# SebLague/Ray-Tracing

Hardware: AMD Instinct MI355X
Metric: Mrays/s at 1920x1080, 8 spp, 8 bounces; per-channel L2 vs reference (higher is better)
Workload: dtype f32

## Files before the change

### ray-tracing_amd/csrc/rt_context.hip

```cpp
#include <hip/hip_runtime.h>

#include <math.h>
#include <stdarg.h>
#include <stdio.h>
#include <stdlib.h>
#include <string.h>
#include <dlfcn.h>
#include <sys/mman.h>

#include <cmath>
#include <string>
#include <vector>

#include <algorithm>
#include <atomic>
#include <chrono>
#include <mutex>
#include <thread>
#include <unordered_map>

#include "rt_kernels.h"
#include "../../include/rt_cost.h"
#include "../../include/rt_aov.h"
#include "../../include/rt_denoise.h"
#include "../../include/rt_reproject.h"

#include "rt_denoise_launch.h"
#include "rt_denoise_math.h"
#include "rt_reproject_launch.h"
#include "rt_layout.h"
#include "rt_launch_order.h"
#include "rt_launch_plan.h"
#define RT_VERSION_STRING "raytrace_hip gfx950 abi=1"

static thread_local char g_err[512] = "";

struct RtContext;
struct LaunchJob;
struct HipOrder final : rt_order::Backend {
    RtContext* ctx = nullptr;
    hipEvent_t ev[rt_order::EVENT_COUNT] = {};
    LaunchJob* job = nullptr;
    hipStream_t stream(int s) const;
    int record(rt_order::Event e, int s) override;
// ... 87 lines not shown
    struct Tuner {
        int decided = 3;
        bool done = false;
        double ms[2] = {0, 0};
        int n[2] = {0, 0};
        int next = 0;
        struct Probe { hipEvent_t start = nullptr, stop = nullptr; int cand = 0, frames = 0; bool live = false; } probe[6];
    } tuner;
    float* dStaging[2] = {nullptr, nullptr};
    size_t stagingBytes[2] = {0, 0};
    bool stagingUnavailable = false;
    bool alternateWanted = true;
    rt_order::LaunchOrder order;
    HipOrder backend;
    int lastLaunched = 0;
    void* dDisplay = nullptr;
    void* dAovOut = nullptr;
    size_t aovOutBytes = 0;
    unsigned long long* dAovWords = nullptr;
    bool aovUnreported = false;
    void* dDnScratch = nullptr;
    size_t dnScratchBytes = 0;
    void* dDnAov = nullptr;
    size_t dnAovBytes = 0;
    size_t displayBytes = 0;
    hipEvent_t evStart = nullptr, evStop = nullptr;
    double gpuMs = 0;
    int timerState = 0;
};

// ... 145 lines not shown
        HIP_TRY(ctx, hipMalloc(&ctx->dTileQueue, 2 * sizeof(unsigned long long)));
        HIP_TRY(ctx, hipMemsetAsync(ctx->dTileQueue, 0, 2 * sizeof(unsigned long long), ctx->ownStream));
        HIP_TRY(ctx, hipStreamSynchronize(ctx->ownStream));
        HIP_TRY(ctx, hipEventCreate(&ctx->evStart));
        HIP_TRY(ctx, hipEventCreate(&ctx->evStop));
        for (hipEvent_t& ev : ctx->backend.ev) HIP_TRY(ctx, hipEventCreateWithFlags(&ev, hipEventDisableTiming));
        return RT_OK;
    };
    if (int rc = init()) {
        rt_destroy(ctx);
        return rc;
    }
    memset(&ctx->params, 0, sizeof(ctx->params));
    if (const char* g = getenv("RT_GRID")) ctx->gridOverride = atoi(g);
    if (const char* g = getenv("RT_POOL_MIN_ITEMS")) ctx->poolMinItems = atoi(g);
    if (const char* g = getenv("RT_POOL_FAULT")) { if (atoi(g)) ctx->poolSpinLimit = 64u | 0x80000000u; }
    if (getenv("RT_VERBOSE")) ctx->verbose = true;
    if (const char* f = getenv("RT_FUSE_FRAMES")) ctx->fuseFrames = atoi(f) != 0;
    if (const char* l = getenv("RT_LPT")) ctx->order.lpt = atoi(l) != 0;
    if (const char* t = getenv("RT_TWO_STREAMS")) ctx->twoStreams = atoi(t) != 0;
    if (const char* c = getenv("RT_COALESCE")) ctx->coalesce = atoi(c) != 0;
    if (const char* fg = getenv("RT_FRAME_GROUP")) ctx->frameGroupOverride = atoi(fg);
    if (const char* al = getenv("RT_ALTERNATE")) ctx->order.alternate = ctx->alternateWanted = atoi(al) != 0;
    ctx->order.set_two_streams(ctx->twoStreams && ctx->sideStream);
    if (const char* fc = getenv("RT_FUSE_CAP"))
        if (const int cap = rt_plan::pinned_fuse_cap(atoi(fc))) { ctx->fuseCap = cap; ctx->fuseCapPinned = true; }
    *out = ctx;
    return RT_OK;
}

// ... 13 lines not shown
    ctx->haveScene = false;
}

void rt_destroy(RtContext* ctx)
{
    if (!ctx) return;
    hipSetDevice(ctx->device);
    flush_pending(ctx);
    if (ctx->sideStream) hipStreamSynchronize(ctx->sideStream);
    hipStreamSynchronize(ctx->stream);
    free_scene(ctx);
    hipFree(ctx->ownFrame);
    hipFree(ctx->ownAccum);
    hipFree(ctx->dCounters);
    hipFree(ctx->dTileQueue);
    hipFree(ctx->dTileCost);
    hipFree(ctx->dTileOrder[0]);
    hipFree(ctx->dTileOrder[1]);
    hipFree(ctx->dTileKey);
    hipFree(ctx->dDisplay);
    hipFree(ctx->dAovOut);
    hipFree(ctx->dAovWords);
    hipFree(ctx->dDnScratch);
    hipFree(ctx->dDnAov);
    hipFree(ctx->dStaging[0]);
    hipFree(ctx->dStaging[1]);
    hipFree(ctx->dPxCold);
    for (auto& pr : ctx->tuner.probe) {
        if (pr.start) hipEventDestroy(pr.start);
        if (pr.stop) hipEventDestroy(pr.stop);
// ... 775 lines not shown
    }
    ctx->wavesPerGroup = ctx->hotUnits ? ps.wavesPerGroup : 1;
    {
        int on = 1, waves = RT_MAX_WAVES_PER_GROUP_FLAT;
        if (const char* e = getenv("RT_POOL")) on = atoi(e);
        if (const char* e = getenv("RT_POOL_WAVES")) waves = atoi(e);
        if (waves < 1) waves = 1;
        if (waves > RT_MAX_WAVES_PER_GROUP_FLAT) waves = RT_MAX_WAVES_PER_GROUP_FLAT;
        const bool pooled = ps.flat && on;
        ctx->poolWaves = pooled ? waves : 1;
        ctx->poolCells = pooled ? (int)RT_POOL_CELLS : 0;
    }
    ctx->hModels = ps.hModels;
    ctx->hRootCodes = ps.rootCodes;
    ctx->haveScene = true;
    ctx->tuner.done = getenv("RT_SUSPEND") != nullptr;
    ctx->tuner.decided = ctx->tuner.done ? atoi(getenv("RT_SUSPEND")) : 3;
    if (ctx->tuner.decided < 1 || ctx->tuner.decided > 7) ctx->tuner.decided = 3;
    ctx->tuner.ms[0] = ctx->tuner.ms[1] = 0;
    ctx->tuner.n[0] = ctx->tuner.n[1] = 0;
    ctx->tuner.next = 0;
    for (auto& pr : ctx->tuner.probe) pr.live = false;
    return RT_OK;
}

extern "C" {

int rt_upload_scene(RtContext* ctx, const RtModel* models, int n_models, const RtTriangle* triangles, int n_triangles,
                    const RtBVHNode* nodes, int n_nodes, const RtSphere* spheres, int n_spheres)
{
// ... 60 lines not shown
    free(d->pair_space); free(d->tri_space); free(d->norm_space); free(d->big_leaves); free(d->root_codes); free(d->tri_base);
    memset(d, 0, sizeof(*d));
}

int rt_update_models(RtContext* ctx, const RtModel* models, int n_models)
{
    if (!ctx) return fail(nullptr, RT_ERR_INVALID_ARG, "null context");
    if (!ctx->haveScene) return fail(ctx, RT_ERR_STATE, "rt_update_models before rt_upload_scene");
    if (n_models != ctx->nModels || (n_models && !models)) return fail(ctx, RT_ERR_INVALID_ARG, "rt_update_models: model count changed (%d != %d)", n_models, ctx->nModels);
    if (n_models == 0) return RT_OK;
    if (memcmp(models, ctx->hModels.data(), sizeof(RtModel) * (size_t)n_models) == 0) {
        ctx->updateSkips++;
        return RT_OK;
    }
    RT_FLUSH(ctx);
    std::vector<DModel> dmodels(n_models);
    std::vector<DMaterial> mats(n_models);
    bool matricesChanged = false;
    for (int i = 0; i < n_models; i++) {
        if (models[i].nodeOffset != ctx->hModels[i].nodeOffset || models[i].triOffset != ctx->hModels[i].triOffset)
            return fail(ctx, RT_ERR_INVALID_ARG, "rt_update_models: model %d changed its BVH offsets; re-upload the scene", i);
        pack_model(models[i], ctx->hRootCodes[i], ctx->hTriBase[i], dmodels[i]);
        pack_material(models[i].material, mats[i]);
        if (memcmp(models[i].worldToLocal, ctx->hModels[i].worldToLocal, sizeof(models[i].worldToLocal)) != 0 ||
            memcmp(models[i].localToWorld, ctx->hModels[i].localToWorld, sizeof(models[i].localToWorld)) != 0)
            matricesChanged = true;
    }
    HIP_TRY(ctx, hipSetDevice(ctx->device));
    int rc;
    if ((rc = stage_upload(ctx, ctx->dModels, dmodels.data(), sizeof(DModel) * n_models))) return rc;
// ... 10 lines not shown
    ctx->hModels.assign(models, models + n_models);
    return RT_OK;
}

int rt_update_spheres(RtContext* ctx, const RtSphere* spheres, int n_spheres)
{
    if (!ctx) return fail(nullptr, RT_ERR_INVALID_ARG, "null context");
    if (!ctx->haveScene) return fail(ctx, RT_ERR_STATE, "rt_update_spheres before rt_upload_scene");
    if (n_spheres != ctx->nSpheres || (n_spheres && !spheres)) return fail(ctx, RT_ERR_INVALID_ARG, "rt_update_spheres: sphere count changed");
    if (n_spheres == 0) return RT_OK;
    if (memcmp(spheres, ctx->hSpheres.data(), sizeof(RtSphere) * (size_t)n_spheres) == 0) {
        ctx->updateSkips++;
        return RT_OK;
    }
    RT_FLUSH(ctx);
    std::vector<float> sph;
    pack_spheres(spheres, n_spheres, sph, &ctx->sphereBound);
    std::vector<DMaterial> mats(n_spheres);
    for (int i = 0; i < n_spheres; i++) pack_material(spheres[i].material, mats[i]);
    HIP_TRY(ctx, hipSetDevice(ctx->device));
    int rc;
    if ((rc = stage_upload(ctx, ctx->dSpheres, sph.data(), sph.size() * 4))) return rc;
    if ((rc = stage_upload(ctx, ctx->dMaterials, mats.data(), sizeof(DMaterial) * n_spheres))) return rc;
    ctx->hSpheres.assign(spheres, spheres + n_spheres);
    if (ctx->nModels) {
        std::vector<DFilter> filters;
        make_filters(ctx->hModels.data(), ctx->nModels, ctx->hRootCodes, ctx->hRootChildren, spheres, n_spheres, filters, &ctx->filterMaxOrigin);
        {
            const std::vector<DFilter> up = append_filter_pairs(filters);
            if ((rc = stage_upload(ctx, ctx->dFilters, up.data(), sizeof(DFilter) * up.size()))) return rc;
// ... 376 lines not shown
    mark_fused_launch_end(ctx, fuseSlot, st, nFrames);
    ctx->tileQueueNext[s] = pp.queueNext;
    return RT_OK;
}

int HipOrder::accumulate(int s)
{
    int blocks = (int)((job->nPix + 255) / 256);
    if (blocks > 4096) blocks = 4096;
    hipLaunchKernelGGL(rtk::rt_accumulate_kernel, dim3(blocks), dim3(256), 0, stream(s), (const float4*)ctx->dStaging[s], job->nFrames, job->nPix,
                       (float4*)job->a.accumulated, (float4*)job->a.frameRender, job->nPix);
    HIP_TRY(ctx, hipGetLastError());
    return RT_OK;
}

static int launch_frames(RtContext* ctx, int frame0, int nFrames)
{
    KArgs a;
    fill_args(ctx, frame0, nFrames, a);
    const int tiles = a.tilesX * a.tilesY;
    if (tiles == 0) return RT_OK;
    LaunchPlan plan;
    int rc = choose_variant(ctx, a, plan);
    if (rc) return rc;
    if ((rc = prepare_records(ctx, plan))) return rc;
    if ((rc = prepare_tile_order(ctx, a, tiles))) return rc;
    rt_order::Shape shape;
    shape.frames = nFrames;
    shape.singleWave = plan.shape.wavesPerGroup == 1;
    shape.tiles = tiles;
    const rt_order::Placement pl = ctx->order.place(shape);
    const size_t nPix = (size_t)ctx->localRows * ctx->W;
    if (pl.staged) {
        bool unavailable = false;
        if ((rc = prepare_staging(ctx, a, nFrames, nPix, pl.lane, pl.split, &unavailable))) return rc;
        if (unavailable) {
// ... 297 lines not shown
    }
    for (int p = 0; p < RT_N_PHASES && 2 * RT_N_PHASES + 1 + p < n; p++) {
        out[2 * RT_N_PHASES + 1 + p] = 0;
        if (p < 3)
            for (int s = 0; s < RT_COUNTER_SLOTS; s++) out[2 * RT_N_PHASES + 1 + p] += h[(size_t)s * RT_COUNTER_FIELDS + 8 + 2 * RT_N_PHASES + p];
    }
    return RT_OK;
}

struct DevScratch {
    void* p = nullptr;
    ~DevScratch() { if (p) hipFree(p); }
    hipError_t alloc(size_t bytes) { return hipMalloc(&p, bytes); }
    float* f() const { return (float*)p; }
};

int rt_debug_fused_frames_cap(const RtContext* ctx) { return ctx ? ctx->fuseCap : RT_ERR_INVALID_ARG; }

int rt_debug_intersect(RtContext* ctx, const float* origins, const float* dirs, int n, float* out10)
{
    if (ctx) RT_FLUSH(ctx);
    if (!ctx) return fail(nullptr, RT_ERR_INVALID_ARG, "null context");
    if (!ctx->haveScene) return fail(ctx, RT_ERR_STATE, "rt_debug_intersect before rt_upload_scene");
    if (n < 0 || (n && (!origins || !dirs || !out10))) return fail(ctx, RT_ERR_INVALID_ARG, "rt_debug_intersect: bad arguments");
    if (n == 0) return RT_OK;
    HIP_TRY(ctx, hipSetDevice(ctx->device));
    DevScratch dO, dD, dR;
    HIP_TRY(ctx, dO.alloc((size_t)n * 12));
    HIP_TRY(ctx, dD.alloc((size_t)n * 12));
    HIP_TRY(ctx, dR.alloc((size_t)n * 40));
// ... 960 lines not shown
```

### ray-tracing_amd/csrc/rt_device.h

```cpp
#ifndef RT_DEVICE_H
#define RT_DEVICE_H

#include <stdint.h>

#include "rt_launch_plan.h"

#define RT_STACK_DEPTH 34
#define RT_COUNTER_SLOTS 1024
#define RT_N_PHASES 12
#define RT_COLD_STRIDE_BYTES (2 * RT_WAVE * 16)
#define RT_COUNTER_FIELDS (8 + 2 * RT_N_PHASES + 4)

#define RT_CODE_LEAF 0x80000000u
#define RT_CODE_NEXT_MODEL 0x7fffffffu
#define RT_CODE_DONE 0x7ffffffeu
#define RT_CODE_MAX_INLINE_COUNT 127
#define RT_CODE_MAX_INLINE_START 0x00ffffffu

struct DPair {
    float aMin[3], aMax[3];
    float bMin[3], bMax[3];
    uint32_t codeA, codeB;
    uint32_t pad[2];
};
// ... 75 lines not shown
    int32_t launchTiles, orderOffset, orderStride;
    int32_t launchItems;
    float4* pxCold;
    int32_t frameGroup;
    int32_t frameGroups;
    float* staging;
    uint32_t stagingStride;
    int32_t queueStart;
    unsigned long long* tileQueue;
    unsigned long long tileQueueBase;
    const uint32_t* tileOrder;
    uint32_t* tileCost;
    int32_t poolCells;
    int32_t frameGroupShift;
    uint32_t poolSpinLimit;
};

#endif
```

### ray-tracing_amd/csrc/rt_kernels.h

```cpp
#ifndef RT_KERNELS_H
#define RT_KERNELS_H

#include <hip/hip_runtime.h>

#include "../../include/rt_abi.h"
#include "../../include/rt_math.h"
#include "rt_device.h"

#ifndef RT_SUSPEND_NUM
#define RT_SUSPEND_NUM 3
#define RT_SUSPEND_DEN 8
#endif
#ifndef RT_INNER_BURST
#define RT_INNER_BURST 3
#endif

namespace rtk {

#define RT_CAS __attribute__((address_space(4)))
#define RT_LDS __attribute__((address_space(3)))

__device__ __forceinline__ float hw_min(float a, float b) { return __builtin_fminf(a, b); }
__device__ __forceinline__ float hw_max(float a, float b) { return __builtin_fmaxf(a, b); }

// ... 713 lines not shown
    }
    if (HOT && !FLAT && hotUnits) {
        const float4* src = reinterpret_cast<const float4*>(a.pairs);
        float4* dst = reinterpret_cast<float4*>(s_lds);
        const uint32_t nHot = hotUnits >> 2;
        for (uint32_t i = threadIdx.x; i < hotUnits; i += blockDim.x) dst[(i & 3u) * nHot + (i >> 2)] = src[i];
        __syncthreads();
    }
    uint32_t* const s_stack = HOT ? s_lds + (hotUnits * 4u + (uint32_t)wave * (uint32_t)a.waveLdsDwords) : s_lds;
    const int gw = HOT ? (int)blockIdx.x * a.wavesPerGroup + wave : (int)blockIdx.x;
    uint32_t* stackBase = &s_stack[lane];

    int poolX0 = 0, poolRow0 = 0, poolY0 = 0;
    int poolPos = 0;
    int poolTile = 0;
    int poolFrame = 0;
#define RT_ITEM(c, q, tilePos)                                  \
    do {                                                        \
        if ((c).nFrames > 1) {                                  \
            tilePos = (q) / (c).frameGroups;                    \
            poolFrame = (c).frame0 + ((q) - tilePos * (c).frameGroups) * (c).frameGroup; \
        } else {                                                \
            tilePos = (q);                                      \
            poolFrame = (c).frame0;                             \
        }                                                       \
    } while (0)
    bool queueEmpty;
#define RT_SET_POOL(c, tile)                                                                              \
    do {                                                                                                  \
        const int ty_ = (tile) / (c).tilesX;                                                              \
        poolX0 = ((tile) - ty_ * (c).tilesX) * 8;                                                         \
        poolRow0 = ty_ * 8;                                                                               \
        const int ls_ = poolRow0 / (c).stripRows;                                                         \
        poolY0 = (ls_ * (c).partCount + (c).partIndex) * (c).stripRows + (poolRow0 - ls_ * (c).stripRows); \
        poolPos = 0;                                                                                      \
        if (FLAT) poolTile = (tile);                                                                      \
    } while (0)
    {
        const RT_CAS KArgs& c = cold_args();
        int tile = gw;
        if (tile < c.launchItems && c.nFrames > 0 && !c.queueStart) {
            const int q0_ = tile;
            RT_ITEM(c, q0_, tile);
            tile = tile * c.orderStride + c.orderOffset;
            if (c.tileOrder) tile = (int)c.tileOrder[tile];
            RT_SET_POOL(c, tile);
        } else {
            poolPos = 64;
        }
        queueEmpty = (c.nFrames <= 0);
    }
// ... 51 lines not shown
                if (x < (int)c.W && lrow < c.localRows) {
                    const int y = poolY0 + (slot >> 3);
                    const float uvx = (float)(uint32_t)x * c.rcpWm1;
                    const float uvy = (float)(uint32_t)y * c.rcpHm1;
                    const uint32_t pixelCoordX = (uint32_t)(uvx * (float)c.W);
                    const uint32_t pixelCoordY = (uint32_t)(uvy * (float)c.H);
                    const uint32_t pixelIndex = pixelCoordY * c.W + pixelCoordX;
                    const rt_f3 fpl = rt_v3(uvx - 0.5f, uvy - 0.5f, 1.0f) * rt_v3(c.viewParams[0], c.viewParams[1], c.viewParams[2]);
                    float cam[16];
                    for (int k = 0; k < 16; k++) cam[k] = c.cam[k];
                    const rt_f3 focusPoint = rt_mul_point(cam, fpl, 1.0f);
                    {
                        float4* const cold = PX_COLD(c);
                        cold[0] = make_float4(focusPoint.x, focusPoint.y, focusPoint.z, __uint_as_float(pixelIndex));
                        cold[RT_WAVE] = make_float4(__uint_as_float((uint32_t)lrow * c.W + (uint32_t)x), __uint_as_float(segments), __uint_as_float((uint32_t)poolFrame),
                                                    FLAT ? __uint_as_float((uint32_t)poolTile) : 0.0f);
                    }
                    PXU(PX_SAMPLE) = 0;
                    PXF(PX_TIX) = 0.0f; PXF(PX_TIY) = 0.0f; PXF(PX_TIZ) = 0.0f;
                    rng = pixelIndex + (uint32_t)poolFrame * 719393u + (uint32_t)c.seed;
                    pathActive = false;
                    inTrav = false;
                    laneDone = false;
                    if constexpr (COST) {
                        uint4* const o = reinterpret_cast<uint4*>(cost) + 2 * (size_t)((uint32_t)lrow * c.W + (uint32_t)x);
                        o[0] = make_uint4(segments, st.inner, st.leaf, st.tri);
                        o[1] = make_uint4(0u, 0u, 0u, 0u);
                    }
                }
            }
            const int wanted = __popcll(idle);
            poolPos += wanted < avail ? wanted : avail;
            idle = __ballot(laneDone);
        }
        if (idle == ~0ull) {
            if (!POOL) break;
            if (RT_RFL(RT_POOL_LOAD(s_lds + 0)) == RT_RFL(RT_POOL_LOAD(s_lds + 3)) && RT_RFL(RT_POOL_LOAD(s_lds + 2)) == RT_RFL(RT_POOL_LOAD(s_lds + 1))) break;
        }
        if (!laneDone) {
        phase_mark<STATS>(st, PH_LOOP);
        if (!inTrav) {
            if (!pathActive) {
                const RT_CAS KArgs& c = cold_args();
                const uint32_t sampleWord = PXU(PX_SAMPLE);
                const bool grouped = FLAT && c.frameGroup > 1;
                int sample = grouped ? (int)(sampleWord & 0xffffu) : (int)sampleWord;
                if (sample == c.spp) {
                    float4* const cold = PX_COLD(c);
                    const float4 rec = cold[RT_WAVE];
                    const uint32_t pixLinear = __float_as_uint(rec.x), segStart = __float_as_uint(rec.y);
                    const int frameFirst = (int)__float_as_uint(rec.z);
                    const int frameNow = frameFirst + (grouped ? (int)(sampleWord >> 16) : 0);
                    const size_t pixOff = (size_t)pixLinear * 4;
                    rt_f3 col = rt_v3(PXF(PX_TIX), PXF(PX_TIY), PXF(PX_TIZ)) * c.rcpSpp;
                    if constexpr (COST) {
                        uint4* const o = reinterpret_cast<uint4*>(cost) + 2 * (size_t)pixLinear;
                        const uint4 s0 = o[0];
                        o[0] = make_uint4(segments - s0.x, st.inner - s0.y, st.leaf - s0.z, st.tri - s0.w);
                    } else if (c.nFrames > 1) {
                        const size_t slab = (size_t)(frameNow - c.frame0) * c.stagingStride;
                        *reinterpret_cast<float4*>(c.staging + (slab + pixLinear) * 4) = make_float4(col.x, col.y, col.z, 1.0f);
                    } else {
                        *reinterpret_cast<float4*>(c.frameRender + pixOff) = make_float4(col.x, col.y, col.z, 1.0f);
                        if (c.accumulate) {
                            float4 acc = *reinterpret_cast<float4*>(c.accumulated + pixOff);
                            acc.x += col.x;
                            acc.y += col.y;
// ... 35 lines not shown
                        rayOrigin = camOrigin;
                    } else {
                        rt_f2 dj = rand_circle(&rng);
                        rayOrigin = camOrigin + camRight * (dj.x * c.defocus * invNumPixelsX) + camUp * (dj.y * c.defocus * invNumPixelsX);
                    }
                    rt_f2 jj = rand_circle(&rng);
                    const float4 fp4 = PX_COLD(c)[0];
                    const rt_f3 focusPoint = rt_v3(fp4.x, fp4.y, fp4.z);
                    rt_f3 jfp = focusPoint + camRight * (jj.x * c.diverge * invNumPixelsX) + camUp * (jj.y * c.diverge * invNumPixelsX);
                    rpos = rayOrigin;
                    rdir = rt_normalize(jfp - rayOrigin);
                    transmittance = rt_v3s(1.0f);
                    pathLight = rt_v3s(0.0f);
                    if (MANY) extBase[(1 + a.extWords) * RT_WAVE] = 0u;
                    else bounce = 0;
                    PXU(PX_SAMPLE) = grouped ? (PXU(PX_SAMPLE) & 0xffff0000u) | (uint32_t)(sample + 1) : (uint32_t)(sample + 1);
                    if (c.maxBounce >= 0) pathActive = true;
                    else { PXF(PX_TIX) = PXF(PX_TIX) + 0.0f; PXF(PX_TIY) = PXF(PX_TIY) + 0.0f; PXF(PX_TIZ) = PXF(PX_TIZ) + 0.0f; }
                    if constexpr (COST) if (pathActive) {
                        uint4* const o = RT_COST_SLOT(c) + 1;
                        uint4 p = *o;
                        p.x -= st.inner; p.y -= st.leaf; p.z -= st.tri;
                        *o = p;
                    }
                }
            }
            if (pathActive) {
                phase_mark<STATS>(st, PH_SPHERES);
                begin_intersect<STATS, FLAT, MANY>(a, rpos, rdir, extBase, h, t, st);
                segments++;
                inTrav = true;
                if (FLAT) traverse_flat<STATS>(a, rpos, rdir, h, st);
            }
        }
        if constexpr (!POOL) {
#include "rt_shade_phase.inl"
        }
        }
        if constexpr (POOL) {
            pool_exchange<STATS>(a, s_lds, lane, pxu, PX_COLD(cold_args()), laneDone, pathActive, inTrav, rpos, rdir, transmittance, pathLight, rng, bounce, h, segments, st);
            if (!laneDone) {
#include "rt_shade_phase.inl"
            }
        }
    }

#undef RT_SET_POOL
// ... 260 lines not shown
```

### ray-tracing_amd/hip.py

```python
import ctypes as C
import os

import numpy as np

from . import abi

_HERE = os.path.dirname(os.path.abspath(__file__))
LIB_PATH = os.environ.get("RT_HIP_LIB") or os.path.join(_HERE, "lib", "libraytrace_hip.so")

ABI_SYMBOLS = [
    "rt_create", "rt_destroy", "rt_last_error", "rt_set_stream", "rt_resize", "rt_set_partition", "rt_local_rows",
    "rt_local_to_global_row", "rt_bind_render_targets", "rt_get_render_targets", "rt_upload_scene", "rt_update_models",
    "rt_update_spheres", "rt_set_params", "rt_reset_accumulation", "rt_render_frame", "rt_render_frames",
    "rt_synchronize", "rt_get_frame", "rt_read_frame", "rt_read_accumulated", "rt_display", "rt_display_srgb8",
    "rt_write_accumulated", "rt_timer_begin", "rt_timer_end",
    "rt_enable_stats", "rt_reset_counters", "rt_get_counters", "rt_build_bvh", "rt_build_bvh_mt", "rt_build_bvh_gpu", "rt_build_bvh_gpu_release", "rt_camera_view_params", "rt_version",
    "rt_debug_intersect", "rt_debug_math_eval", "rt_debug_phase_profile", "rt_build_bvh_gpu_batch",
    "rt_flush", "rt_validate_scene", "rt_debug_layout", "rt_debug_layout_free", "rt_debug_fused_frames_cap",
    "rt_create_multi", "rt_destroy_multi", "rt_multi_count", "rt_multi_context", "rt_multi_resize", "rt_multi_upload_scene",
    "rt_multi_update_models", "rt_multi_update_spheres", "rt_multi_set_params", "rt_multi_reset_accumulation",
    "rt_multi_render_frame", "rt_multi_render_frames", "rt_multi_synchronize", "rt_gather_accumulated", "rt_gather_frame",
    "rt_multi_get_counters", "rt_multi_last_gather_ms", "rt_multi_peer_access", "rt_gather_accumulated_to_device", "rt_gather_frame_to_device",
    "rt_gather_rccl",
]
COST_SYMBOLS = ["rt_render_cost"]
AOV_SYMBOLS = ["rt_render_aov", "rt_render_aov_to_device"]
DENOISE_SYMBOLS = ["rt_denoise_default_params", "rt_denoise_buffers", "rt_denoise", "rt_denoise_to_device"]
REPROJECT_SYMBOLS = ["rt_reproject_default_params", "rt_reproject_buffers", "rt_reproject_accumulated", "rt_resolve_buffers", "rt_resolve",
                     "rt_resolve_to_device"]
COST_FIELDS = ("segments", "innerSteps", "leafSteps", "triTests", "primaryInnerSteps", "primaryLeafSteps", "primaryTriTests", "firstHit")


class HipApi(abi.CApi):
    _EXTRA = {
        "create": (C.c_int, [C.c_int, C.POINTER(C.c_void_p)]),
        "set_stream": (C.c_int, [C.c_void_p, C.c_void_p]),
        "set_partition": (C.c_int, [C.c_void_p, C.c_int, C.c_int, C.c_int]),
        "local_rows": (C.c_int, [C.c_void_p]),
        "local_to_global_row": (C.c_int, [C.c_void_p, C.c_int]),
        "bind_render_targets": (C.c_int, [C.c_void_p, C.c_void_p, C.c_void_p]),
        "get_render_targets": (C.c_int, [C.c_void_p, C.POINTER(C.c_void_p), C.POINTER(C.c_void_p)]),
        "synchronize": (C.c_int, [C.c_void_p]),
        "flush": (C.c_int, [C.c_void_p]),
        "timer_begin": (C.c_int, [C.c_void_p]),
        "timer_end": (C.c_int, [C.c_void_p]),
        "enable_stats": (C.c_int, [C.c_void_p, C.c_int]),
        "build_bvh_mt": (C.c_int, [C.c_void_p, C.c_void_p, C.c_int, C.c_void_p, C.c_int, C.c_int, C.c_int, C.c_void_p,
                                   C.POINTER(C.c_int), C.c_void_p, C.POINTER(abi.RtBvhStats)]),
        "build_bvh_gpu": (C.c_int, [C.c_int, C.c_void_p, C.c_void_p, C.c_int, C.c_void_p, C.c_int, C.c_int, C.c_void_p,
                                    C.POINTER(C.c_int), C.c_void_p, C.POINTER(abi.RtBvhStats)]),
        "build_bvh_gpu_release": (None, []),
        "build_bvh_gpu_batch": (C.c_int, [C.c_int, C.c_int, C.c_void_p, C.c_void_p, C.c_void_p, C.c_void_p, C.c_void_p, C.c_int, C.c_void_p,
                                          C.c_void_p, C.c_void_p, C.c_void_p, C.c_void_p, C.c_void_p]),
        "validate_scene": (C.c_int, [C.c_void_p, C.c_int, C.c_void_p, C.c_int, C.c_void_p, C.c_int, C.c_void_p, C.c_int, C.c_void_p]),
        "debug_layout": (C.c_int, [C.c_void_p, C.c_int, C.c_void_p, C.c_int, C.c_void_p, C.c_int, C.c_char_p, C.c_void_p]),
        "debug_layout_free": (None, [C.c_void_p]),
        "debug_fused_frames_cap": (C.c_int, [C.c_void_p]),
        "debug_intersect": (C.c_int, [C.c_void_p, C.c_void_p, C.c_void_p, C.c_int, C.c_void_p]),
        "debug_math_eval": (C.c_int, [C.c_void_p, C.c_int, C.c_void_p, C.c_void_p, C.c_void_p, C.c_int]),
        "debug_phase_profile": (C.c_int, [C.c_void_p, C.c_void_p, C.c_int]),
        "create_multi": (C.c_int, [C.POINTER(C.c_int), C.c_int, C.POINTER(C.c_void_p)]),
        "destroy_multi": (None, [C.c_void_p]),
        "multi_count": (C.c_int, [C.c_void_p]),
        "multi_context": (C.c_void_p, [C.c_void_p, C.c_int]),
        "multi_resize": (C.c_int, [C.c_void_p, C.c_int, C.c_int]),
        "multi_upload_scene": (C.c_int, [C.c_void_p, C.c_void_p, C.c_int, C.c_void_p, C.c_int, C.c_void_p, C.c_int, C.c_void_p, C.c_int]),
        "multi_update_models": (C.c_int, [C.c_void_p, C.c_void_p, C.c_int]),
        "multi_update_spheres": (C.c_int, [C.c_void_p, C.c_void_p, C.c_int]),
        "multi_set_params": (C.c_int, [C.c_void_p, C.POINTER(abi.RtParams)]),
        "multi_reset_accumulation": (C.c_int, [C.c_void_p]),
        "multi_render_frame": (C.c_int, [C.c_void_p]),
        "multi_render_frames": (C.c_int, [C.c_void_p, C.c_int]),
# ... 301 lines not shown

    def bind_render_targets(self, frame_ptr, accum_ptr):
        self._check(self.api.bind_render_targets(self.h, frame_ptr, accum_ptr))

    def render_targets(self):
        f, a = C.c_void_p(), C.c_void_p()
        self._check(self.api.get_render_targets(self.h, C.byref(f), C.byref(a)))
        return f.value, a.value

    def gather_rccl(self, nccl_comm, root, device_ptr, nbytes, accumulated=True):
        self._check(self.api.gather_rccl(self.h, nccl_comm, int(root), 1 if accumulated else 0, device_ptr, nbytes))

    def fused_frames_cap(self):
        return self.api.debug_fused_frames_cap(self.h)

    def synchronize(self):
        self._check(self.api.synchronize(self.h))

    def flush(self):
        self._check(self.api.flush(self.h))

    def timer_begin(self):
        self._check(self.api.timer_begin(self.h))

    def timer_end(self):
        self._check(self.api.timer_end(self.h))

    def enable_stats(self, on=True):
        self._check(self.api.enable_stats(self.h, 1 if on else 0))

# ... 92 lines not shown
```

Before: 47520.

## Skip primary-ray traversal for tiles whose view frustum misses all scene geometry

Adds a conservative per-tile classifier kernel. It builds a padded double-precision frustum for each 8x8 tile and tests every sphere and model bounding box against it, marking tiles that cannot be hit by any primary ray. The flag is packed into the sample word's top bit, and the flat render kernel skips begin_intersect/traverse_flat on bounce 0 for flagged tiles. The classification is cached against a key of camera, tiling and scene epoch, so it reruns only when these change. The cost is extra bit-masking in the hot path and a small risk of wrong results if the conservative bounds are ever too tight.

```diff
diff --git a/include/rt_tile_class.h b/include/rt_tile_class.h
--- /dev/null
+++ b/include/rt_tile_class.h
@@ -0,0 +1,18 @@
+#ifndef RT_TILE_CLASS_H
+#define RT_TILE_CLASS_H
+
+#include "rt_abi.h"
+
+#ifdef __cplusplus
+extern "C" {
+#endif
+
+int rt_debug_tile_classes(RtContext* ctx, uint8_t* out, size_t n);
+
+int rt_debug_tile_class_runs(const RtContext* ctx);
+
+#ifdef __cplusplus
+}
+#endif
+
+#endif
diff --git a/ray-tracing_amd/csrc/rt_context.hip b/ray-tracing_amd/csrc/rt_context.hip
--- a/ray-tracing_amd/csrc/rt_context.hip
+++ b/ray-tracing_amd/csrc/rt_context.hip
@@ -24,10 +24,12 @@
 #include "../../include/rt_aov.h"
 #include "../../include/rt_denoise.h"
 #include "../../include/rt_reproject.h"
+#include "../../include/rt_tile_class.h"
 
 #include "rt_denoise_launch.h"
 #include "rt_denoise_math.h"
 #include "rt_reproject_launch.h"
+#include "rt_tile_class_launch.h"
 #include "rt_layout.h"
 #include "rt_launch_order.h"
 #include "rt_launch_plan.h"
@@ -145,6 +147,17 @@
     rt_order::LaunchOrder order;
     HipOrder backend;
     int lastLaunched = 0;
+    struct TileKey {
+        rt_tc_view view;
+        rt_tc::Tiles tiles;
+        uint64_t sceneEpoch;
+    } tileKey;
+    bool tileKeyValid = false;
+    bool tileSkip = true;
+    uint64_t sceneEpoch = 0;
+    uint64_t tileClassRuns = 0;
+    unsigned char* dTileClass = nullptr;
+    int tileClassBytes = 0;
     void* dDisplay = nullptr;
     void* dAovOut = nullptr;
     size_t aovOutBytes = 0;
@@ -320,6 +333,7 @@
     memset(&ctx->params, 0, sizeof(ctx->params));
     if (const char* g = getenv("RT_GRID")) ctx->gridOverride = atoi(g);
     if (const char* g = getenv("RT_POOL_MIN_ITEMS")) ctx->poolMinItems = atoi(g);
+    if (const char* g = getenv("RT_TILE_SKIP")) ctx->tileSkip = atoi(g) != 0;
     if (const char* g = getenv("RT_POOL_FAULT")) { if (atoi(g)) ctx->poolSpinLimit = 64u | 0x80000000u; }
     if (getenv("RT_VERBOSE")) ctx->verbose = true;
     if (const char* f = getenv("RT_FUSE_FRAMES")) ctx->fuseFrames = atoi(f) != 0;
@@ -363,6 +377,7 @@
     hipFree(ctx->ownAccum);
     hipFree(ctx->dCounters);
     hipFree(ctx->dTileQueue);
+    hipFree(ctx->dTileClass);
     hipFree(ctx->dTileCost);
     hipFree(ctx->dTileOrder[0]);
     hipFree(ctx->dTileOrder[1]);
@@ -1168,6 +1183,7 @@
     ctx->hModels = ps.hModels;
     ctx->hRootCodes = ps.rootCodes;
     ctx->haveScene = true;
+    ctx->sceneEpoch++;
     ctx->tuner.done = getenv("RT_SUSPEND") != nullptr;
     ctx->tuner.decided = ctx->tuner.done ? atoi(getenv("RT_SUSPEND")) : 3;
     if (ctx->tuner.decided < 1 || ctx->tuner.decided > 7) ctx->tuner.decided = 3;
@@ -1258,6 +1274,7 @@
         return RT_OK;
     }
     RT_FLUSH(ctx);
+    ctx->sceneEpoch++;
     std::vector<DModel> dmodels(n_models);
     std::vector<DMaterial> mats(n_models);
     bool matricesChanged = false;
@@ -1298,6 +1315,7 @@
         return RT_OK;
     }
     RT_FLUSH(ctx);
+    ctx->sceneEpoch++;
     std::vector<float> sph;
     pack_spheres(spheres, n_spheres, sph, &ctx->sphereBound);
     std::vector<DMaterial> mats(n_spheres);
@@ -1704,12 +1722,60 @@
     return RT_OK;
 }
 
+static int ensure_tile_classes(RtContext* ctx, KArgs& a)
+{
+    if (!ctx->flatScene) return RT_OK;
+    const int tiles = a.tilesX * a.tilesY;
+    RtContext::TileKey key;
+    memset(&key, 0, sizeof(key));
+    memcpy(key.view.cam, a.cam, sizeof(a.cam));
+    memcpy(key.view.viewParams, a.viewParams, sizeof(a.viewParams));
+    key.view.diverge = a.diverge;
+    key.view.rcpW = a.rcpW;
+    key.view.rcpWm1 = a.rcpWm1;
+    key.view.rcpHm1 = a.rcpHm1;
+    key.view.filterMaxOrigin = a.filterMaxOrigin;
+    key.view.raygenNoDefocus = a.raygenNoDefocus;
+    key.view.maxBounce = a.maxBounce;
+    key.view.enabled = ctx->tileSkip ? 1 : 0;
+    key.tiles.tiles = tiles;
+    key.tiles.tilesX = a.tilesX;
+    key.tiles.bytes = (tiles + 3) & ~3;
+    key.tiles.W = (int)a.W;
+    key.tiles.localRows = a.localRows;
+    key.tiles.stripRows = a.stripRows;
+    key.tiles.partIndex = a.partIndex;
+    key.tiles.partCount = a.partCount;
+    key.sceneEpoch = ctx->sceneEpoch;
+    if (!ctx->tileKeyValid || memcmp(&key, &ctx->tileKey, sizeof(key)) != 0) {
+        ctx->tileKeyValid = false;
+        if (ctx->tileClassBytes < key.tiles.bytes) {
+            HIP_TRY(ctx, hipStreamSynchronize(joined(ctx)));
+            hipFree(ctx->dTileClass); ctx->dTileClass = nullptr; ctx->tileClassBytes = 0;
+            HIP_TRY(ctx, hipMalloc(&ctx->dTileClass, (size_t)key.tiles.bytes));
+            ctx->tileClassBytes = key.tiles.bytes;
+        }
+        rt_tc::Scene sc;
+        sc.spheres = ctx->dSpheres;
+        sc.filters = ctx->dFilters;
+        sc.nSpheres = ctx->nSpheres;
+        sc.nModels = ctx->nModels;
+        HIP_TRY(ctx, rt_tc::enqueue(joined(ctx), key.view, sc, key.tiles, ctx->dTileClass));
+        memcpy(&ctx->tileKey, &key, sizeof(key));
+        ctx->tileKeyValid = true;
+        ctx->tileClassRuns++;
+    }
+    a.tileClass = reinterpret_cast<const uint32_t*>(ctx->dTileClass);
+    return RT_OK;
+}
+
 static int launch_frames(RtContext* ctx, int frame0, int nFrames)
 {
     KArgs a;
     fill_args(ctx, frame0, nFrames, a);
     const int tiles = a.tilesX * a.tilesY;
     if (tiles == 0) return RT_OK;
+    if (int rc = ensure_tile_classes(ctx, a)) return rc;
     LaunchPlan plan;
     int rc = choose_variant(ctx, a, plan);
     if (rc) return rc;
@@ -2037,6 +2103,29 @@
     hipError_t alloc(size_t bytes) { return hipMalloc(&p, bytes); }
     float* f() const { return (float*)p; }
 };
+
+int rt_debug_tile_classes(RtContext* ctx, uint8_t* out, size_t n)
+{
+    int rc = check_renderable(ctx);
+    if (rc) return rc;
+    RT_FLUSH(ctx);
+    HIP_TRY(ctx, hipSetDevice(ctx->device));
+    KArgs a;
+    fill_args(ctx, ctx->frame, 1, a);
+    const size_t tiles = (size_t)a.tilesX * a.tilesY;
+    if (!out || n != tiles) return fail(ctx, RT_ERR_INVALID_ARG, "rt_debug_tile_classes: %zu entries given, the context has %zu tiles", n, tiles);
+    if (tiles == 0) return RT_OK;
+    if ((rc = ensure_tile_classes(ctx, a))) return rc;
+    if (!a.tileClass) {
+        memset(out, 0, tiles);
+        return RT_OK;
+    }
+    HIP_TRY(ctx, hipStreamSynchronize(joined(ctx)));
+    HIP_TRY(ctx, hipMemcpy(out, ctx->dTileClass, tiles, hipMemcpyDeviceToHost));
+    return RT_OK;
+}
+
+int rt_debug_tile_class_runs(const RtContext* ctx) { return ctx ? (int)ctx->tileClassRuns : RT_ERR_INVALID_ARG; }
 
 int rt_debug_fused_frames_cap(const RtContext* ctx) { return ctx ? ctx->fuseCap : RT_ERR_INVALID_ARG; }
 
diff --git a/ray-tracing_amd/csrc/rt_device.h b/ray-tracing_amd/csrc/rt_device.h
--- a/ray-tracing_amd/csrc/rt_device.h
+++ b/ray-tracing_amd/csrc/rt_device.h
@@ -113,6 +113,7 @@
     int32_t poolCells;
     int32_t frameGroupShift;
     uint32_t poolSpinLimit;
+    const uint32_t* tileClass;
 };
 
 #endif
diff --git a/ray-tracing_amd/csrc/rt_kernels.h b/ray-tracing_amd/csrc/rt_kernels.h
--- a/ray-tracing_amd/csrc/rt_kernels.h
+++ b/ray-tracing_amd/csrc/rt_kernels.h
@@ -751,6 +751,7 @@
     int poolX0 = 0, poolRow0 = 0, poolY0 = 0;
     int poolPos = 0;
     int poolTile = 0;
+    constexpr bool SKIP = FLAT && !STATS && !COST;
     int poolFrame = 0;
 #define RT_ITEM(c, q, tilePos)                                  \
     do {                                                        \
@@ -771,7 +772,12 @@
         const int ls_ = poolRow0 / (c).stripRows;                                                         \
         poolY0 = (ls_ * (c).partCount + (c).partIndex) * (c).stripRows + (poolRow0 - ls_ * (c).stripRows); \
         poolPos = 0;                                                                                      \
-        if (FLAT) poolTile = (tile);                                                                      \
+        if (FLAT) {                                                                                       \
+             \
+            const RT_CAS uint32_t* const tc_ = (const RT_CAS uint32_t*)(c).tileClass;                     \
+            poolTile = (tile);                                                                            \
+            if (tc_ && ((tc_[(tile) >> 2] >> (((tile) & 3) * 8)) & 1u)) poolTile |= (int)0x80000000u;     \
+        }                                                                                                 \
     } while (0)
     {
         const RT_CAS KArgs& c = cold_args();
@@ -853,9 +859,9 @@
                         float4* const cold = PX_COLD(c);
                         cold[0] = make_float4(focusPoint.x, focusPoint.y, focusPoint.z, __uint_as_float(pixelIndex));
                         cold[RT_WAVE] = make_float4(__uint_as_float((uint32_t)lrow * c.W + (uint32_t)x), __uint_as_float(segments), __uint_as_float((uint32_t)poolFrame),
-                                                    FLAT ? __uint_as_float((uint32_t)poolTile) : 0.0f);
+                                                    FLAT ? __uint_as_float((uint32_t)poolTile & 0x7fffffffu) : 0.0f);
                     }
-                    PXU(PX_SAMPLE) = 0;
+                    PXU(PX_SAMPLE) = FLAT ? (uint32_t)poolTile & 0x80000000u : 0u;
                     PXF(PX_TIX) = 0.0f; PXF(PX_TIY) = 0.0f; PXF(PX_TIZ) = 0.0f;
                     rng = pixelIndex + (uint32_t)poolFrame * 719393u + (uint32_t)c.seed;
                     pathActive = false;
@@ -883,13 +889,13 @@
                 const RT_CAS KArgs& c = cold_args();
                 const uint32_t sampleWord = PXU(PX_SAMPLE);
                 const bool grouped = FLAT && c.frameGroup > 1;
-                int sample = grouped ? (int)(sampleWord & 0xffffu) : (int)sampleWord;
+                int sample = grouped ? (int)(sampleWord & 0xffffu) : (int)(FLAT ? sampleWord & 0x7fffffffu : sampleWord);
                 if (sample == c.spp) {
                     float4* const cold = PX_COLD(c);
                     const float4 rec = cold[RT_WAVE];
                     const uint32_t pixLinear = __float_as_uint(rec.x), segStart = __float_as_uint(rec.y);
                     const int frameFirst = (int)__float_as_uint(rec.z);
-                    const int frameNow = frameFirst + (grouped ? (int)(sampleWord >> 16) : 0);
+                    const int frameNow = frameFirst + (grouped ? (int)((sampleWord >> 16) & 0x7fffu) : 0);
                     const size_t pixOff = (size_t)pixLinear * 4;
                     rt_f3 col = rt_v3(PXF(PX_TIX), PXF(PX_TIY), PXF(PX_TIZ)) * c.rcpSpp;
                     if constexpr (COST) {
@@ -955,7 +961,7 @@
                     pathLight = rt_v3s(0.0f);
                     if (MANY) extBase[(1 + a.extWords) * RT_WAVE] = 0u;
                     else bounce = 0;
-                    PXU(PX_SAMPLE) = grouped ? (PXU(PX_SAMPLE) & 0xffff0000u) | (uint32_t)(sample + 1) : (uint32_t)(sample + 1);
+                    PXU(PX_SAMPLE) = grouped ? (PXU(PX_SAMPLE) & 0xffff0000u) | (uint32_t)(sample + 1) : (FLAT ? sampleWord & 0x80000000u : 0u) | (uint32_t)(sample + 1);
                     if (c.maxBounce >= 0) pathActive = true;
                     else { PXF(PX_TIX) = PXF(PX_TIX) + 0.0f; PXF(PX_TIY) = PXF(PX_TIY) + 0.0f; PXF(PX_TIZ) = PXF(PX_TIZ) + 0.0f; }
                     if constexpr (COST) if (pathActive) {
@@ -966,12 +972,29 @@
                     }
                 }
             }
+            if constexpr (SKIP) {
+                if (pathActive) {
+                    const bool run = !(bounce == 0 && (PXU(PX_SAMPLE) >> 31));
+                    h.dst = RT_INF; h.obj = -1; h.tri = -1; h.u = h.v = h.det = 0.0f; h.backface = false;
+                    if (__ballot(run) != 0ull) {
+                        if (run) {
+                            begin_intersect<STATS, FLAT, MANY>(a, rpos, rdir, extBase, h, t, st);
+                            traverse_flat<STATS>(a, rpos, rdir, h, st);
+                        }
+                    }
+                    segments++;
+                    inTrav = true;
+                }
+            } else
             if (pathActive) {
                 phase_mark<STATS>(st, PH_SPHERES);
                 begin_intersect<STATS, FLAT, MANY>(a, rpos, rdir, extBase, h, t, st);
                 segments++;
                 inTrav = true;
                 if (FLAT) traverse_flat<STATS>(a, rpos, rdir, h, st);
+                if constexpr (FLAT && STATS) {
+                    if (bounce == 0 && (PXU(PX_SAMPLE) >> 31) && h.obj >= 0) st.filterViolations++;
+                }
             }
         }
         if constexpr (!POOL) {
diff --git a/ray-tracing_amd/csrc/rt_tile_class.hip b/ray-tracing_amd/csrc/rt_tile_class.hip
--- /dev/null
+++ b/ray-tracing_amd/csrc/rt_tile_class.hip
@@ -0,0 +1,35 @@
+#include <hip/hip_runtime.h>
+
+#include "rt_tile_class_launch.h"
+
+namespace rt_tc {
+
+__global__ __launch_bounds__(256) void rt_tile_class_kernel(const rt_tc_view view, const Scene sc, const Tiles tl, unsigned char* __restrict__ out)
+{
+    const int tile = (int)(blockIdx.x * 256u + threadIdx.x);
+    if (tile >= tl.bytes) return;
+    unsigned char flag = 0;
+    if (tile < tl.tiles) {
+        const rt_tc_rect r = rt_tc_tile_rect(tile, tl.tilesX, tl.W, tl.localRows, tl.stripRows, tl.partIndex, tl.partCount);
+        if (r.any) {
+            const rt_tc_cone cone = rt_tc_make_cone(view, r.x0, r.x1, r.y0, r.y1);
+            bool empty = cone.ok;
+            for (int s = 0; empty && s < sc.nSpheres; s++) empty = rt_tc_sphere_outside(cone, sc.spheres + 4 * s, sc.spheres[4 * s + 3]);
+            for (int m = 0; empty && m < sc.nModels; m++) {
+                const DFilter& f = sc.filters[m];
+                empty = !f.always && rt_tc_box_outside(cone, f.bMin, f.bMax);
+            }
+            flag = empty ? 1 : 0;
+        }
+    }
+    out[tile] = flag;
+}
+
+hipError_t enqueue(hipStream_t st, const rt_tc_view& view, const Scene& sc, const Tiles& tl, unsigned char* dOut)
+{
+    if (tl.bytes <= 0) return hipSuccess;
+    hipLaunchKernelGGL(rt_tile_class_kernel, dim3((unsigned)((tl.bytes + 255) / 256)), dim3(256), 0, st, view, sc, tl, dOut);
+    return hipGetLastError();
+}
+
+}
diff --git a/ray-tracing_amd/csrc/rt_tile_class_launch.h b/ray-tracing_amd/csrc/rt_tile_class_launch.h
--- /dev/null
+++ b/ray-tracing_amd/csrc/rt_tile_class_launch.h
@@ -0,0 +1,27 @@
+#ifndef RT_TILE_CLASS_LAUNCH_H
+#define RT_TILE_CLASS_LAUNCH_H
+
+#include <hip/hip_runtime.h>
+
+#include "rt_device.h"
+#include "rt_tile_class_math.h"
+
+namespace rt_tc {
+
+struct Scene {
+    const float* spheres;
+    const DFilter* filters;
+    int nSpheres, nModels;
+};
+
+struct Tiles {
+    int tiles, tilesX;
+    int bytes;
+    int W, localRows, stripRows, partIndex, partCount;
+};
+
+hipError_t enqueue(hipStream_t st, const rt_tc_view& view, const Scene& sc, const Tiles& tl, unsigned char* dOut);
+
+}
+
+#endif
diff --git a/ray-tracing_amd/csrc/rt_tile_class_math.h b/ray-tracing_amd/csrc/rt_tile_class_math.h
--- /dev/null
+++ b/ray-tracing_amd/csrc/rt_tile_class_math.h
@@ -0,0 +1,189 @@
+#ifndef RT_TILE_CLASS_MATH_H
+#define RT_TILE_CLASS_MATH_H
+
+#include "../../include/rt_math.h"
+
+struct rt_tc_view {
+    float cam[16];
+    float viewParams[3];
+    float diverge, rcpW;
+    float rcpWm1, rcpHm1;
+    float filterMaxOrigin;
+    int raygenNoDefocus, maxBounce;
+    int enabled;
+};
+
+#define RT_TC_PLANES 32
+
+struct rt_tc_cone {
+    double pl[RT_TC_PLANES][3];
+    double o[3];
+    double n[5][3];
+    double slope;
+    bool ok;
+};
+
+RT_HD bool rt_tc_fin(double x) { return x - x == 0.0; }
+RT_HD double rt_tc_abs(double x) { return x < 0.0 ? -x : x; }
+RT_HD double rt_tc_dot(const double* a, const double* b) { return a[0] * b[0] + a[1] * b[1] + a[2] * b[2]; }
+RT_HD void rt_tc_cross(const double* a, const double* b, double* c)
+{
+    c[0] = a[1] * b[2] - a[2] * b[1];
+    c[1] = a[2] * b[0] - a[0] * b[2];
+    c[2] = a[0] * b[1] - a[1] * b[0];
+}
+RT_HD double rt_tc_sqrt(double x) { return __builtin_sqrt(x); }
+
+RT_HD bool rt_tc_view_ok(const rt_tc_view& v)
+{
+    if (!v.enabled || !v.raygenNoDefocus || v.maxBounce < 0) return false;
+    double sum = 0.0;
+    for (int k = 0; k < 16; k++) sum += rt_tc_abs((double)v.cam[k]);
+    sum += rt_tc_abs((double)v.viewParams[0]) + rt_tc_abs((double)v.viewParams[1]) + rt_tc_abs((double)v.viewParams[2]);
+    sum += rt_tc_abs((double)v.diverge) + rt_tc_abs((double)v.rcpW) + rt_tc_abs((double)v.rcpWm1) + rt_tc_abs((double)v.rcpHm1) + rt_tc_abs((double)v.filterMaxOrigin);
+    if (!rt_tc_fin(sum)) return false;
+    for (int k = 12; k < 15; k++)
+        if (!(rt_tc_abs((double)v.cam[k]) <= (double)v.filterMaxOrigin)) return false;
+    return true;
+}
+
+RT_HD rt_tc_cone rt_tc_make_cone(const rt_tc_view& v, int x0, int x1, int y0, int y1)
+{
+    rt_tc_cone c;
+    c.ok = false;
+    c.slope = 0.0;
+    for (int k = 0; k < 3; k++) c.o[k] = (double)v.cam[12 + k];
+    for (int i = 0; i < 5; i++) c.n[i][0] = c.n[i][1] = c.n[i][2] = 0.0;
+    for (int i = 0; i < RT_TC_PLANES; i++) c.pl[i][0] = c.pl[i][1] = c.pl[i][2] = 0.0;
+    if (!rt_tc_view_ok(v)) return c;
+    const double R[3] = {(double)v.cam[0], (double)v.cam[1], (double)v.cam[2]};
+    const double U[3] = {(double)v.cam[4], (double)v.cam[5], (double)v.cam[6]};
+    const double F[3] = {(double)v.cam[8], (double)v.cam[9], (double)v.cam[10]};
+    const double vp0 = (double)v.viewParams[0], vp1 = (double)v.viewParams[1], vp2 = (double)v.viewParams[2];
+    double aLo = ((double)x0 * (double)v.rcpWm1 - 0.5) * vp0, aHi = ((double)x1 * (double)v.rcpWm1 - 0.5) * vp0;
+    double bLo = ((double)y0 * (double)v.rcpHm1 - 0.5) * vp1, bHi = ((double)y1 * (double)v.rcpHm1 - 0.5) * vp1;
+    if (aLo > aHi) { const double t = aLo; aLo = aHi; aHi = t; }
+    if (bLo > bHi) { const double t = bLo; bLo = bHi; bHi = t; }
+    const double s = rt_tc_abs((double)v.diverge * (double)v.rcpW) * (1.0 + 1e-6);
+    aLo -= s + 1e-6 * rt_tc_abs(vp0); aHi += s + 1e-6 * rt_tc_abs(vp0);
+    bLo -= s + 1e-6 * rt_tc_abs(vp1); bHi += s + 1e-6 * rt_tc_abs(vp1);
+    if (!(aHi > aLo && bHi > bLo)) return c;
+    double pn[3];
+    rt_tc_cross(R, U, pn);
+    const double pnLen = rt_tc_sqrt(rt_tc_dot(pn, pn));
+    if (!(pnLen > 0.0)) return c;
+    const double L = rt_tc_abs(rt_tc_dot(pn, F) * vp2) / pnLen;
+    const double lenR = rt_tc_sqrt(rt_tc_dot(R, R)), lenU = rt_tc_sqrt(rt_tc_dot(U, U)), lenF = rt_tc_sqrt(rt_tc_dot(F, F));
+    const double aMax = rt_tc_abs(aLo) > rt_tc_abs(aHi) ? rt_tc_abs(aLo) : rt_tc_abs(aHi);
+    const double bMax = rt_tc_abs(bLo) > rt_tc_abs(bHi) ? rt_tc_abs(bLo) : rt_tc_abs(bHi);
+    const double M = rt_tc_sqrt(rt_tc_dot(c.o, c.o)) + lenF * rt_tc_abs(vp2) + lenR * aMax + lenU * bMax;
+    const double u = 5.9604644775390625e-08;
+    if (!(L > 0.0)) return c;
+    const double theta = 1e-4 + 2.0 * (32.0 * u * M) / L + 16.0 * u;
+    if (!(theta < 1e-2)) return c;
+    c.slope = theta + theta * theta;
+    const double ca[4] = {aLo, aHi, aHi, aLo}, cb[4] = {bLo, bLo, bHi, bHi};
+    double d[4][3], mid[3] = {0.0, 0.0, 0.0};
+    for (int k = 0; k < 4; k++)
+        for (int j = 0; j < 3; j++) {
+            d[k][j] = F[j] * vp2 + R[j] * ca[k] + U[j] * cb[k];
+            mid[j] += 0.25 * d[k][j];
+        }
+    for (int i = 0; i < 4; i++) {
+        double n[3];
+        rt_tc_cross(d[i], d[(i + 1) & 3], n);
+        const double len = rt_tc_sqrt(rt_tc_dot(n, n));
+        if (!(len > 0.0) || !rt_tc_fin(len)) return c;
+        const double sgn = rt_tc_dot(n, mid) > 0.0 ? -1.0 : 1.0;
+        for (int j = 0; j < 3; j++) c.n[i][j] = sgn * n[j] / len;
+        if (!(rt_tc_dot(c.n[i], d[(i + 2) & 3]) < 0.0 && rt_tc_dot(c.n[i], d[(i + 3) & 3]) < 0.0)) return c;
+    }
+    const double midLen = rt_tc_sqrt(rt_tc_dot(mid, mid));
+    if (!(midLen > 0.0) || !rt_tc_fin(midLen)) return c;
+    for (int j = 0; j < 3; j++) c.n[4][j] = -mid[j] / midLen;
+    for (int k = 0; k < 4; k++)
+        if (!(rt_tc_dot(c.n[4], d[k]) < 0.0)) return c;
+    for (int idx = 0; idx < RT_TC_PLANES; idx++) {
+        const int side = idx & 3, step = idx >> 2;
+        const double w = (double)step * 0.125;
+        const double* a = c.n[(side + 3) & 3];
+        const double* b = c.n[side];
+        double n[3];
+        for (int j = 0; j < 3; j++) n[j] = w * a[j] + (1.0 - w) * b[j];
+        const double len = rt_tc_sqrt(rt_tc_dot(n, n));
+        if (!(len > 0.0)) return c;
+        for (int j = 0; j < 3; j++) c.pl[idx][j] = n[j] / len;
+    }
+    c.ok = true;
+    return c;
+}
+
+RT_HD bool rt_tc_sphere_outside(const rt_tc_cone& c, const float* centre, float r2)
+{
+    if (!c.ok) return false;
+    const double p[3] = {(double)centre[0] - c.o[0], (double)centre[1] - c.o[1], (double)centre[2] - c.o[2]};
+    const double pp = rt_tc_dot(p, p);
+    const double u = 5.9604644775390625e-08;
+    const double rr = rt_tc_abs((double)r2) * (1.0 + 32.0 * u) + 64.0 * u * pp;
+    const double reach = rt_tc_sqrt(rr) + c.slope * rt_tc_sqrt(pp);
+    if (!rt_tc_fin(reach)) return false;
+    if (rt_tc_dot(c.n[4], p) > reach) return true;
+    for (int i = 0; i < RT_TC_PLANES; i++)
+        if (rt_tc_dot(c.pl[i], p) > reach) return true;
+    return false;
+}
+
+RT_HD bool rt_tc_box_outside(const rt_tc_cone& c, const float* bMin, const float* bMax)
+{
+    if (!c.ok) return false;
+    double p[8][3], back[8], big = 0.0;
+    for (int k = 0; k < 8; k++) {
+        p[k][0] = (double)((k & 1) ? bMax[0] : bMin[0]) - c.o[0];
+        p[k][1] = (double)((k & 2) ? bMax[1] : bMin[1]) - c.o[1];
+        p[k][2] = (double)((k & 4) ? bMax[2] : bMin[2]) - c.o[2];
+        const double len = rt_tc_sqrt(rt_tc_dot(p[k], p[k]));
+        big = len > big ? len : big;
+        back[k] = rt_tc_dot(c.n[4], p[k]);
+        if (!rt_tc_fin(len)) return false;
+    }
+    const double lim = c.slope * big;
+    if (!rt_tc_fin(lim)) return false;
+    bool anyFront = false;
+    for (int k = 0; k < 8; k++) anyFront = anyFront || !(back[k] > lim);
+    if (!anyFront) return true;
+    for (int i = 0; i < RT_TC_PLANES; i++) {
+        const double* n = c.pl[i];
+        bool all = true;
+        for (int k = 0; k < 8 && all; k++) {
+            if (back[k] > lim) continue;
+            if (!(rt_tc_dot(n, p[k]) > lim)) all = false;
+            for (int a = 0; a < 3 && all; a++) {
+                const int j = k ^ (1 << a);
+                if (!(back[j] > lim)) continue;
+                const double t = (lim - back[k]) / (back[j] - back[k]);
+                const double q[3] = {p[k][0] + t * (p[j][0] - p[k][0]), p[k][1] + t * (p[j][1] - p[k][1]), p[k][2] + t * (p[j][2] - p[k][2])};
+                if (!(rt_tc_dot(n, q) > lim)) all = false;
+            }
+        }
+        if (all) return true;
+    }
+    return false;
+}
+
+struct rt_tc_rect { int x0, x1, y0, y1; bool any; };
+RT_HD rt_tc_rect rt_tc_tile_rect(int tile, int tilesX, int W, int localRows, int stripRows, int partIndex, int partCount)
+{
+    rt_tc_rect r;
+    const int ty = tile / tilesX;
+    r.x0 = (tile - ty * tilesX) * 8;
+    const int row0 = ty * 8;
+    const int ls = row0 / stripRows;
+    r.y0 = (ls * partCount + partIndex) * stripRows + (row0 - ls * stripRows);
+    const int nx = W - r.x0 < 8 ? W - r.x0 : 8, ny = localRows - row0 < 8 ? localRows - row0 : 8;
+    r.any = nx > 0 && ny > 0;
+    r.x1 = r.x0 + nx - 1;
+    r.y1 = r.y0 + ny - 1;
+    return r;
+}
+
+#endif
diff --git a/ray-tracing_amd/hip.py b/ray-tracing_amd/hip.py
--- a/ray-tracing_amd/hip.py
+++ b/ray-tracing_amd/hip.py
@@ -28,6 +28,7 @@
 DENOISE_SYMBOLS = ["rt_denoise_default_params", "rt_denoise_buffers", "rt_denoise", "rt_denoise_to_device"]
 REPROJECT_SYMBOLS = ["rt_reproject_default_params", "rt_reproject_buffers", "rt_reproject_accumulated", "rt_resolve_buffers", "rt_resolve",
                      "rt_resolve_to_device"]
+TILE_CLASS_SYMBOLS = ["rt_debug_tile_classes", "rt_debug_tile_class_runs"]
 COST_FIELDS = ("segments", "innerSteps", "leafSteps", "triTests", "primaryInnerSteps", "primaryLeafSteps", "primaryTriTests", "firstHit")
 
 
@@ -56,6 +57,8 @@
         "debug_layout": (C.c_int, [C.c_void_p, C.c_int, C.c_void_p, C.c_int, C.c_void_p, C.c_int, C.c_char_p, C.c_void_p]),
         "debug_layout_free": (None, [C.c_void_p]),
         "debug_fused_frames_cap": (C.c_int, [C.c_void_p]),
+        "debug_tile_classes": (C.c_int, [C.c_void_p, C.c_void_p, C.c_size_t]),
+        "debug_tile_class_runs": (C.c_int, [C.c_void_p]),
         "debug_intersect": (C.c_int, [C.c_void_p, C.c_void_p, C.c_void_p, C.c_int, C.c_void_p]),
         "debug_math_eval": (C.c_int, [C.c_void_p, C.c_int, C.c_void_p, C.c_void_p, C.c_void_p, C.c_int]),
         "debug_phase_profile": (C.c_int, [C.c_void_p, C.c_void_p, C.c_int]),
@@ -387,6 +390,14 @@
     def fused_frames_cap(self):
         return self.api.debug_fused_frames_cap(self.h)
 
+    def tile_classes(self):
+        out = np.zeros(((max(self.local_rows(), 0) + 7) // 8, (self.width + 7) // 8), dtype=np.uint8)
+        self._check(self.api.debug_tile_classes(self.h, out.ctypes.data if out.size else None, out.size))
+        return out
+
+    def tile_class_runs(self):
+        return self.api.debug_tile_class_runs(self.h)
+
     def synchronize(self):
         self._check(self.api.synchronize(self.h))
 
```

Measured after the change: 51470 (median of 6 runs). +8.3%, better.
